# Eun0/XMC-GAN

Hardware: AMD Instinct MI355X
Metric: images/sec per G+D step (higher is better)
Workload: dtype bf16; 1 GPU; 256x256 COCO-shaped synthetic batch, 256 images per GPU, one full G+D iteration (D step + G step + Adam x2), df_gan_damsm_nomagp.yml; per_gpu_batch=256, global_batch=256, image_size=256, cfg=df_gan_damsm_nomagp.yml, parallelism=dp1, hipgraph=True, losses_finite=True, workload_name=headline

## Files before the change

### include/xmc_gan_hip.h

```cpp
#ifndef XMC_GAN_HIP_H
#define XMC_GAN_HIP_H

#include <stdint.h>

#ifdef __cplusplus
extern "C" {
#endif

#define XMC_ABI_VERSION 12

enum { XMC_BF16 = 0, XMC_F32 = 1 };
enum { XMC_HALF_IS_BF16 = 0, XMC_HALF_IS_F16 = 1 };
enum { XMC_ACT_NONE = 0, XMC_ACT_LRELU = 1, XMC_ACT_TANH = 2, XMC_ACT_RELU = 3 };
enum { XMC_EINVAL = -1, XMC_EALIGN = -2, XMC_ESHAPE = -3 };

#define XMC_MAX_TAPS 16
#define XMC_MAX_CLASSES 4

typedef struct XmcConvDesc {
    const void* src;
    const void* wpk;
    void* dst;
    const float* bias;
    const void* res;
// ... 38 lines not shown
const char* xmc_last_kernel(void);
int xmc_set_fixed_order(int on);
int xmc_set_prezeroed(int on);

int64_t xmc_conv_splitk_ws_bytes(const XmcConvDesc* d);

int xmc_conv_igemm(const XmcConvDesc* d, void* stream);

int xmc_conv_wgrad(const XmcConvDesc* d , float* dwp, void* stream);
#define XMC_BIAS_REPLICAS 16
int xmc_conv_wgrad_bias(const XmcConvDesc* d, float* dwp, float* dbias, void* stream);

int xmc_pack_weight(const float* w, void* wpk, int Co, int Ci, int KH, int KW, int rows_pad, int cols_pad,
                    int transpose , int dtype, const int32_t* row_perm , void* stream);
int xmc_pack_weight_grouped(const float* w, void* wpk, int Co, int Ci, int KH, int KW, int rows_pad, int cols_pad, int transpose,
                            int dtype, const int32_t* row_perm, int groups, void* stream);
int xmc_unpack_wgrad_grouped(const float* dwp, float* gw, int Co, int Ci, int KH, int KW, int rows_pad, int cols_pad,
                             const float* scale_dev, const int32_t* row_perm, int accumulate, int groups, void* stream);
#define XMC_PACK_MULTI_MAX 48
typedef struct XmcPackJob {
    const float* w;
    void* wpk;
    const int32_t* row_perm;
    int32_t Co, Ci, KHW, rows_pad, cols_pad, transpose, dtype, groups, upconv;
    int32_t lo;
} XmcPackJob;
int xmc_pack_weight_multi(const XmcPackJob* jobs , int njobs, void* stream);
int xmc_pack_weight_upconv(const float* w, void* wpk, int Co, int Ci, int rows_pad, int cols_pad, int transpose, int dtype,
                           void* stream);
int xmc_unpack_wgrad(const float* dwp, float* gw, int Co, int Ci, int KH, int KW, int rows_pad, int cols_pad,
                     const float* scale_dev, const int32_t* row_perm, int accumulate, void* stream);
int xmc_unpack_wgrad_bias(const float* dwp, float* gw, int Co, int Ci, int KH, int KW, int rows_pad, int cols_pad,
                          const float* scale_dev, const int32_t* row_perm, int accumulate,
                          const float* gb_replicas, float* gb, int CD, void* stream);
int xmc_unpack_wgrad_bias_dot(const float* dwp, float* gw, int Co, int Ci, int KH, int KW, int rows_pad, int cols_pad,
                              const float* scale_dev, const int32_t* row_perm, int accumulate,
                              const float* gb_replicas, float* gb, int CD, const float* bias_dot, float* dot, void* stream);

int xmc_nchw_to_nhwc8(const float* src , void* dst , int N, int C, int H, int W,
                      int dtype, void* stream);
int xmc_nhwc8_to_nchw(const void* src , float* dst , int N, int C, int H, int W,
                      int dtype, void* stream);

int xmc_lrelu(const void* x, void* y, int64_t n, float slope, int dtype, void* stream);
int xmc_lrelu_mask(const void* dy, const void* ref, void* dx, int64_t n, float slope, int dtype, void* stream);
int xmc_tanh(const void* x, void* y, int64_t n, int dtype, void* stream);
int xmc_signmask_apply(const void* dy, const void* bits, void* dx, int64_t n, float slope, int dtype, void* stream);
int xmc_conv_pw1x1_masked_src(const XmcConvDesc* d, const void* src_bits, void* src_masked, float slope, void* stream);
int xmc_conv_pw1x1_split(const XmcConvDesc* d, void* stream);
int xmc_conv_ptile_bits(const XmcConvDesc* d, void* stream);
int xmc_conv_ptile_scimg(const XmcConvDesc* d, void* stream);
int xmc_conv_wgrad_bits(const XmcConvDesc* d, float* dwp, void* stream);
int xmc_tanh_bwd(const void* dy, const void* y, void* dx, int64_t n, int dtype, void* stream);
int xmc_axpby(const void* a, const void* b, const float* alpha_dev, void* y, int64_t n, int dtype, void* stream);
int xmc_axpby_up(const void* a, const void* b, const float* alpha_dev, void* y, int N, int H, int W, int C, int dtype, void* stream);
int xmc_axpby_up_lrelu(const void* a, const void* b, const float* alpha_dev, void* y, int N, int H, int W, int C, int dtype, void* stream);
int xmc_scale(const void* x, const float* alpha_dev, void* y, int64_t n, int dtype, void* stream);
int xmc_dot(const void* a, const void* b, float* out, int64_t n, int dtype, void* stream);
enum { XMC_GP_BIAS = 1, XMC_GP_RELU = 2, XMC_GP_MASK = 4, XMC_GP_ATOMIC = 8 };
typedef struct XmcGemmProblem {
    const float* A;
    const float* B;
    const float* bias;
    const float* mask;
    float* C;
    float* rowsum;
    int32_t M, N, K;
    int32_t sa_i, sa_r, sb_j, sb_r;
    int32_t flags;
    int32_t tile0;
    int32_t reserved;
} XmcGemmProblem;
int xmc_gemm_group(const XmcGemmProblem* problems, int nproblems, void* stream);
int xmc_embedding_gather(const int64_t* ids, const float* table, float* out, int64_t n_tokens, int dim, int64_t vocab, void* stream);
int xmc_gru_bidir(const float* xproj, const float* w_hh, const float* b_hn, const int32_t* lens, float* words, float* sent, int B, int T,
                  int H, void* stream);
int xmc_lstm_bidir(const float* xproj, const float* w_hh, const int32_t* lens, float* words, float* sent, int B, int T, int H,
                   void* stream);
int xmc_spectral_sigma(const float* W, float* u, float* v, float* scratch, float* sig, float* w_eff, int R, int C, int training,
                       float eps, void* stream);
int xmc_spectral_bwd(const float* g, const float* W, const float* u, const float* v, const float* sig, float* dot, float* dW,
                     int R, int C, void* stream);
int xmc_scale_mask_dot(const void* dy, const void* ref, const float* alpha_dev, void* g, float* dot, int64_t n, int dtype, void* stream);
int xmc_axpby_bwd(const void* dy, const void* b, const float* alpha_dev, void* db, void* da, float* dot,
                  int N, int H, int W, int C, int up, const void* ymask , int dtype, void* stream);
int xmc_colsum(const void* x, float* out, int64_t rows, int C, int dtype, void* stream);
int xmc_avgpool2(const void* x, void* y, int N, int H, int W, int C, int dtype, void* stream);
int xmc_upsample2(const void* x, void* y, int N, int H, int W, int C, float scale, int dtype, void* stream);
int xmc_sumpool2(const void* x, void* y, int N, int H, int W, int C, float scale, int dtype, void* stream);
int xmc_global_avgpool(const void* x, void* y, int N, int HW, int C, int dtype, int out_dtype, void* stream);
int xmc_global_avgpool_bwd(const void* dy, void* dx, int N, int HW, int C, int dtype, int in_dtype, void* stream);

int xmc_affine2_lrelu_fwd(const void* x, const float* g0, const float* b0, const float* g1, const float* b1,
                          void* y, int N, int HW, int C, int dtype, void* stream);
int xmc_affine2_lrelu_bwd(const void* x, const void* dy, const float* g0, const float* b0, const float* g1,
                          const float* b1, void* dx, float* dg0, float* db0, float* dg1, float* db1,
                          int N, int HW, int C, int dtype, void* stream);

int xmc_affine2_act_fwd(const void* x, const float* g0, const float* b0, const float* g1, const float* b1,
                        void* y, int N, int HW, int C, float slope, int dtype, void* stream);
int xmc_affine2_act_bwd(const void* x, const void* dy, const float* g0, const float* b0, const float* g1,
                        const float* b1, void* dx, float* dg0, float* db0, float* dg1, float* db1,
                        int N, int HW, int C, float slope, int dtype, void* stream);
int xmc_affine2_act_bwd_acc(const void* x, const void* dy, const float* g0, const float* b0, const float* g1,
                            const float* b1, void* dx, float* dg0, float* db0, float* dg1, float* db1, const void* dx_in,
                            int N, int HW, int C, float slope, int dtype, void* stream);
// ... 131 lines not shown
```

### xmc-gan_amd/lib.py

```python
import ctypes as C
import os

HERE = os.path.dirname(os.path.abspath(__file__))
LIB_PATH = os.environ.get("XMC_LIB_PATH", os.path.join(HERE, "libxmc_gan_hip.so"))
LIB_PATH_F16 = os.environ.get("XMC_LIB_PATH_F16", os.path.join(HERE, "libxmc_gan_hip_f16.so"))
ABI_VERSION = 12

BF16, F32 = 0, 1
H16 = BF16
ACT_NONE, ACT_LRELU, ACT_TANH, ACT_RELU = 0, 1, 2, 3
MAX_TAPS, MAX_CLASSES = 16, 4

vp, i32, i64, f32 = C.c_void_p, C.c_int32, C.c_int64, C.c_float


class ConvDesc(C.Structure):
    _fields_ = [("src", vp), ("wpk", vp), ("dst", vp), ("bias", vp), ("res", vp), ("alpha_dev", vp),
                ("N", i32), ("SH", i32), ("SW", i32), ("CS", i32),
                ("DH", i32), ("DW", i32), ("CD", i32),
                ("MH", i32), ("MW", i32), ("SA", i32), ("DA", i32), ("src_shift", i32),
                ("ntaps", i32), ("nclass", i32), ("CDw", i32), ("act", i32), ("dtype", i32), ("out_dtype", i32),
                ("dh", (C.c_int8 * MAX_TAPS) * MAX_CLASSES), ("dw", (C.c_int8 * MAX_TAPS) * MAX_CLASSES),
                ("wi", (C.c_int8 * MAX_TAPS) * MAX_CLASSES),
                ("dph", C.c_int8 * MAX_CLASSES), ("dpw", C.c_int8 * MAX_CLASSES),
# ... 2 lines not shown
                ("splitk_ws", vp), ("splitk_ws_bytes", C.c_int64), ("wpk_lo", vp)]


GEMM_PROBLEM = [("A", "u8"), ("B", "u8"), ("bias", "u8"), ("mask", "u8"), ("C", "u8"), ("rowsum", "u8"),
                ("M", "i4"), ("N", "i4"), ("K", "i4"), ("sa_i", "i4"), ("sa_r", "i4"), ("sb_j", "i4"), ("sb_r", "i4"),
                ("flags", "i4"), ("tile0", "i4"), ("reserved", "i4")]
GP_BIAS, GP_RELU, GP_MASK, GP_ATOMIC = 1, 2, 4, 8


class PackJob(C.Structure):
    _fields_ = [("w", vp), ("wpk", vp), ("row_perm", vp), ("Co", i32), ("Ci", i32), ("KHW", i32), ("rows_pad", i32),
                ("cols_pad", i32), ("transpose", i32), ("dtype", i32), ("groups", i32), ("upconv", i32), ("lo", i32)]


class AdamEntry(C.Structure):
    _fields_ = [("param", vp), ("grad", vp), ("m", vp), ("v", vp), ("step", vp), ("n", i64)]


class EmaEntry(C.Structure):
    _fields_ = [("shadow", vp), ("param", vp), ("n", i64)]


_SIGS = {
    "xmc_abi_version": [],
    "xmc_half_format": [],
    "xmc_last_kernel": [],
    "xmc_set_fixed_order": [i32],
    "xmc_set_prezeroed": [i32],
    "xmc_conv_splitk_ws_bytes": [vp],
    "xmc_conv_igemm": [C.POINTER(ConvDesc), vp],
    "xmc_conv_wgrad": [C.POINTER(ConvDesc), vp, vp],
    "xmc_conv_wgrad_bias": [C.POINTER(ConvDesc), vp, vp, vp],
    "xmc_pack_weight": [vp, vp, i32, i32, i32, i32, i32, i32, i32, i32, vp, vp],
    "xmc_pack_weight_grouped": [vp, vp, i32, i32, i32, i32, i32, i32, i32, i32, vp, i32, vp],
    "xmc_pack_weight_upconv": [vp, vp, i32, i32, i32, i32, i32, i32, vp],
    "xmc_pack_weight_multi": [C.POINTER(PackJob), i32, vp],
    "xmc_axpby_up": [vp, vp, vp, vp, i32, i32, i32, i32, i32, vp],
    "xmc_unpack_wgrad": [vp, vp, i32, i32, i32, i32, i32, i32, vp, vp, i32, vp],
    "xmc_unpack_wgrad_grouped": [vp, vp, i32, i32, i32, i32, i32, i32, vp, vp, i32, i32, vp],
    "xmc_unpack_wgrad_bias": [vp, vp, i32, i32, i32, i32, i32, i32, vp, vp, i32, vp, vp, i32, vp],
    "xmc_unpack_wgrad_bias_dot": [vp, vp, i32, i32, i32, i32, i32, i32, vp, vp, i32, vp, vp, i32, vp, vp, vp],
    "xmc_nchw_to_nhwc8": [vp, vp, i32, i32, i32, i32, i32, vp],
    "xmc_nhwc8_to_nchw": [vp, vp, i32, i32, i32, i32, i32, vp],
    "xmc_lrelu": [vp, vp, i64, f32, i32, vp],
    "xmc_lrelu_mask": [vp, vp, vp, i64, f32, i32, vp],
    "xmc_tanh": [vp, vp, i64, i32, vp],
    "xmc_signmask_apply": [vp, vp, vp, i64, f32, i32, vp],
    "xmc_conv_pw1x1_masked_src": [C.POINTER(ConvDesc), vp, vp, f32, vp],
    "xmc_conv_pw1x1_split": [C.POINTER(ConvDesc), vp],
    "xmc_conv_ptile_bits": [C.POINTER(ConvDesc), vp],
    "xmc_conv_ptile_scimg": [C.POINTER(ConvDesc), vp],
    "xmc_conv_wgrad_bits": [C.POINTER(ConvDesc), vp, vp],
    "xmc_tanh_bwd": [vp, vp, vp, i64, i32, vp],
    "xmc_axpby": [vp, vp, vp, vp, i64, i32, vp],
    "xmc_scale_mask_dot": [vp, vp, vp, vp, vp, i64, i32, vp],
    "xmc_axpby_bwd": [vp, vp, vp, vp, vp, vp, i32, i32, i32, i32, i32, vp, i32, vp],
    "xmc_axpby_up_lrelu": [vp, vp, vp, vp, i32, i32, i32, i32, i32, vp],
    "xmc_scale": [vp, vp, vp, i64, i32, vp],
    "xmc_dot": [vp, vp, vp, i64, i32, vp],
    "xmc_gemm_group": [vp, i32, vp],
    "xmc_embedding_gather": [vp, vp, vp, i64, i32, i64, vp],
    "xmc_lstm_bidir": [vp, vp, vp, vp, vp, i32, i32, i32, vp],
    "xmc_gru_bidir": [vp, vp, vp, vp, vp, vp, i32, i32, i32, vp],
    "xmc_spectral_sigma": [vp, vp, vp, vp, vp, vp, i32, i32, i32, f32, vp],
    "xmc_spectral_bwd": [vp, vp, vp, vp, vp, vp, vp, i32, i32, vp],
    "xmc_colsum": [vp, vp, i64, i32, i32, vp],
    "xmc_avgpool2": [vp, vp, i32, i32, i32, i32, i32, vp],
    "xmc_upsample2": [vp, vp, i32, i32, i32, i32, f32, i32, vp],
    "xmc_sumpool2": [vp, vp, i32, i32, i32, i32, f32, i32, vp],
    "xmc_global_avgpool": [vp, vp, i32, i32, i32, i32, i32, vp],
    "xmc_global_avgpool_bwd": [vp, vp, i32, i32, i32, i32, i32, vp],
    "xmc_affine2_act_fwd": [vp, vp, vp, vp, vp, vp, i32, i32, i32, f32, i32, vp],
    "xmc_affine2_act_bwd": [vp, vp, vp, vp, vp, vp, vp, vp, vp, vp, vp, i32, i32, i32, f32, i32, vp],
    "xmc_affine2_act_bwd_acc": [vp, vp, vp, vp, vp, vp, vp, vp, vp, vp, vp, vp, i32, i32, i32, f32, i32, vp],
    "xmc_affine2_act_bwd_dot": [vp, vp, vp, vp, vp, vp, vp, vp, vp, vp, vp, vp, vp, vp, i32, i32, i32, f32, i32, vp],
    "xmc_affine2_act_bwd_dot_pool": [vp, vp, vp, vp, vp, vp, vp, vp, vp, vp, vp, vp, vp, vp, vp, i32, i32, i32, i32, f32, i32, vp],
    "xmc_affine2_lrelu_fwd": [vp, vp, vp, vp, vp, vp, i32, i32, i32, i32, vp],
    "xmc_affine2_lrelu_bwd": [vp, vp, vp, vp, vp, vp, vp, vp, vp, vp, vp, i32, i32, i32, i32, vp],
    "xmc_groupnorm_fwd": [vp, vp, vp, vp, vp, vp, i32, i32, i32, i32, f32, f32, i32, vp],
    "xmc_groupnorm_bwd": [vp, vp, vp, vp, vp, vp, vp, vp, vp, i32, i32, i32, i32, f32, i32, vp],
    "xmc_attn_pool_ws_floats": [i32, i32],
    "xmc_attn_pool_fwd": [vp, vp, vp, vp, vp, vp, i32, i32, i32, i32, i32, f32, i32, vp],
    "xmc_attn_pool_bwd": [vp, vp, vp, vp, vp, vp, vp, vp, vp, i32, i32, i32, i32, i32, f32, i32, vp],
    "xmc_attn_pool_bwd_acc": [vp, vp, vp, vp, vp, vp, vp, vp, vp, vp, i32, i32, i32, i32, i32, f32, i32, vp],
    "xmc_word_pool_fwd": [vp, vp, vp, vp, i32, i32, i32, i32, i32, i32, vp],
    "xmc_word_pool_bwd": [vp, vp, vp, vp, vp, vp, i32, i32, i32, i32, i32, i32, vp],
    "xmc_gvec_fwd": [vp, vp, vp, vp, vp, i32, i32, i32, i32, i32, vp],
    "xmc_gvec_bwd": [vp, vp, vp, vp, vp, vp, vp, vp, i32, i32, i32, i32, i32, vp],
    "xmc_reasoner_fwd": [vp, vp, vp, vp, vp, vp, i32, f32, f32, vp, vp, vp, i32, vp],
    "xmc_reasoner_bwd": [vp, vp, vp, vp, vp, vp, i32, vp, vp, vp, vp, vp, i32, vp],
    "xmc_word_ctx_fwd": [vp, vp, vp, vp, vp, i32, i32, vp],
    "xmc_word_ctx_bwd": [vp, vp, vp, vp, vp, vp, i32, i32, vp],
    "xmc_word_keys_fwd": [vp, vp, vp, f32, vp, vp, i32, i32, vp],
    "xmc_word_keys_bwd": [vp, vp, vp, vp, vp, vp, vp, vp, i32, i32, vp],
    "xmc_contrastive_ws_bytes": [i32, i32],
    "xmc_contrastive_fwd": [vp, vp, vp, vp, i32, i32, vp, vp, vp],
    "xmc_contrastive_bwd": [vp, vp, vp, vp, i32, i32, vp, vp, vp, vp, vp],
    "xmc_cosine_scores": [vp, vp, i32, i32, vp, vp, vp],
    "xmc_hinge_fwd": [vp, i32, f32, vp, i64, i32, vp],
    "xmc_hinge_bwd": [vp, i32, f32, vp, vp, i64, i32, vp],
    "xmc_cast": [vp, vp, i64, i32, i32, vp],
    "xmc_concept_query_fwd": [vp, vp, vp, vp, vp, vp, i32, i32, f32, vp],
    "xmc_concept_query_bwd": [vp, vp, vp, vp, vp, vp, vp, vp, vp, vp, i32, i32, f32, vp],
    "xmc_concept_query_fwd_multi": [vp, vp, vp, vp, i32, vp, vp, i32, i32, f32, vp],
    "xmc_concept_query_bwd_multi": [vp, vp, vp, i32, vp, vp, vp, vp, vp, vp, i32, i32, f32, vp],
    "xmc_concept_gquery_fwd": [vp, vp, vp, vp, vp, vp, i32, f32, vp],
# ... 83 lines not shown
```

### xmc-gan_amd/ops/_engine.py

```python
import ctypes as C
import weakref
import torch
from .. import lib as L
from .. import prof
from ._config import (
    _DEBUG_DISPATCH, _code, _nbytes, _need_cuda, _p, _st, _weights_epoch, bump_weights_epoch, chan_pad, pad_to)


class ConvGeom:

    __slots__ = ("cin", "cout", "k", "s", "p", "row_perm", "_perm_dev", "groups")

    def __init__(self, cin, cout, k=1, s=1, p=0, row_perm=None, groups=1):
        assert k * k <= L.MAX_TAPS and k % s == 0
        assert cin % groups == 0 and cout % groups == 0
        self.cin, self.cout, self.k, self.s, self.p = cin, cout, k, s, p
        self.groups = groups
        self.row_perm = row_perm
        self._perm_dev = None

    def out_hw(self, h, w):
        return (h + 2 * self.p - self.k) // self.s + 1, (w + 2 * self.p - self.k) // self.s + 1

    def perm_dev(self, device):
# ... 506 lines not shown

def _pool_key(t):
    return (t.data_ptr(), tuple(t.shape), t.dtype)


def _pooled_put(dx, dxp):
    _pooled_grads[_pool_key(dx)] = (dx, dx._version, dxp)


def _pooled_take(dz):
    ent = _pooled_grads.pop(_pool_key(dz), None)
    if ent is None:
        return None
    dx, ver, dxp = ent
    same = dx.untyped_storage().data_ptr() == dz.untyped_storage().data_ptr() and dx.stride() == dz.stride() and dx._version == ver
    return dxp if same else None


def _conv_wgrad_raw(x, dy, geom, scale=None, up=False, want_bias=False, bias_dot=None, dot=None):
    staged = dy if isinstance(dy, _StagedMask) else None
    if staged is not None:
        dy = staged.dy
    _need_cuda(x, dy)
    N, H, W, CS = x.shape
    _, OH, OW, CDy = dy.shape
    assert x.dtype == dy.dtype, (x.dtype, dy.dtype)
    rows = pad_to(CDy, 32)
    dwp = _arena.zeros((geom.k * geom.k, rows, CS), x.device)
    gb = _arena.zeros((16, CDy), x.device) if want_bias else None
    d = L.ConvDesc()
    d.src, d.dst = x.data_ptr(), dy.data_ptr()
    d.N, d.SH, d.SW, d.CS = N, H, W, CS
    d.DH, d.DW, d.CD = OH, OW, CDy
    d.MH, d.MW, d.SA, d.DA, d.src_shift = OH, OW, geom.s, 1, 1 if up else 0
    d.ntaps, d.nclass, d.CDw = geom.k * geom.k, 1, rows
    d.dtype, d.out_dtype = _code(x.dtype), L.F32
    d.groups = geom.groups
    _fill_taps(d, 0, [(kh - geom.p, kw - geom.p, kh * geom.k + kw) for kh in range(geom.k) for kw in range(geom.k)])
    rc = 1
    if staged is not None and not want_bias:
        d.mask_bits = staged.bits.data_ptr()
        with prof.launch("wgrad_kernel (conv weight gradient, MFMA + split-K atomics)", 2.0 * N * OH * OW * geom.cout * geom.cin * geom.k * geom.k,
                         f"wgrad+bits {x.dtype} N{N} {H}x{W} {geom.cin}->{geom.cout} k{geom.k}s{geom.s}", _nbytes(x, dy, dwp)):
            rc = L.load().xmc_conv_wgrad_bits(C.byref(d), _p(dwp), _st())
        if rc not in (0, 1):
            L.check(rc, "xmc_conv_wgrad_bits")
        d.mask_bits = None
    if rc == 1:
        if staged is not None:
            d.dst = staged.materialised().data_ptr()
        with prof.launch("wgrad_kernel (conv weight gradient, MFMA + split-K atomics)", 2.0 * N * OH * OW * geom.cout * geom.cin * geom.k * geom.k,
                         f"wgrad {x.dtype} N{N} {H}x{W} {geom.cin}->{geom.cout} k{geom.k}s{geom.s}", _nbytes(x, dy, dwp)):
            L.check(L.load().xmc_conv_wgrad_bias(C.byref(d), _p(dwp), _p(gb), _st()), "xmc_conv_wgrad")
    gw = torch.empty((geom.cout, geom.cin // geom.groups, geom.k, geom.k), dtype=torch.float32, device=x.device)
    if want_bias:
        assert geom.groups == 1
        gbs = torch.empty(CDy, dtype=torch.float32, device=x.device)
        assert (bias_dot is None) == (dot is None)
        L.call("xmc_unpack_wgrad_bias_dot", _p(dwp), _p(gw), geom.cout, geom.cin, geom.k, geom.k, rows, CS, _p(scale),
               _p(geom.perm_dev(x.device)), 0, _p(gb), _p(gbs), CDy, _p(bias_dot), _p(dot), _st())
        return gw, gbs
    assert bias_dot is None
    L.call("xmc_unpack_wgrad_grouped", _p(dwp), _p(gw), geom.cout, geom.cin, geom.k, geom.k, rows, CS, _p(scale),
           _p(geom.perm_dev(x.device)), 0, geom.groups, _st())
    return gw


def _axpby_bwd_fused(dy, b, alpha, up, ymask=None, want_db=True):
    dy = dy.contiguous()
    N, OH, OW, Cc = dy.shape
    H, W = (OH // 2, OW // 2) if up else (OH, OW)
    al = alpha.detach().reshape(-1).float()
    db = torch.empty_like(dy) if want_db else None
    da = torch.empty((N, H, W, Cc), dtype=dy.dtype, device=dy.device) if (up or ymask is not None) else None
    dot = _zeros_f32_out(1, dy.device)
    L.call("xmc_axpby_bwd", _p(dy), _p(b), _p(al), _p(db), _p(da), _p(dot), N, H, W, Cc, 1 if up else 0, _p(ymask), _code(dy.dtype), _st())
    return da, db, dot.reshape(alpha.shape).to(alpha.dtype)


def _affine_fwd_raw(x, ps, slope):
    N, H, W, Cc = x.shape
    for t in ps:
        assert t.shape == (N, Cc), (t.shape, (N, Cc))
    y = torch.empty_like(x)
    ptrs = [_p(t) for t in ps] + ([] if len(ps) == 4 else [None, None])
    L.call("xmc_affine2_act_fwd", _p(x), *ptrs, _p(y), N, H * W, Cc, float(slope), _code(x.dtype), _st())
    return y


def _affine_bwd_raw(x, dy, ps, slope, dx_acc=None, alpha=None, dot=None, want_sumpool=False):
    N, H, W, Cc = x.shape
    dx = torch.empty_like(x)
    if dx_acc is not None:
        dx_acc = dx_acc.contiguous()
        assert dx_acc.shape == x.shape and dx_acc.dtype == x.dtype
    nred = len(ps)
    red = _zeros_f32((nred, N, Cc), x.device)
    ptrs = [_p(t) for t in ps] + ([] if nred == 4 else [None, None])
    rptrs = [_p(red[i]) for i in range(nred)] + ([] if nred == 4 else [None, None])
    assert (alpha is None) == (dot is None)
    dxp = torch.empty((N, H // 2, W // 2, Cc), dtype=x.dtype, device=x.device) if want_sumpool else None
    L.call("xmc_affine2_act_bwd_dot_pool", _p(x), _p(dy), *ptrs, _p(dx), *rptrs, _p(dx_acc), _p(alpha), _p(dot), _p(dxp), N, H, W, Cc,
           float(slope), _code(x.dtype), _st())
    return (dx, red, dxp) if want_sumpool else (dx, red)


def compose_dstem(w_img, b_img, w0, ws, bs):
    F = torch.nn.functional
    co, mid = w0.shape[0], w0.shape[1]
    w0, b_img = w0.float(), b_img.float()
    wie = F.pad(w_img.float(), (0, 0, 0, 0, 0, 8 - w_img.shape[1]))
    wa = F.conv_transpose2d(w0, wie)
    box = torch.full((1, 1, 2, 2), 0.25, dtype=torch.float32, device=w_img.device)
    wp = F.conv_transpose2d(wie.reshape(mid * 8, 1, 3, 3), box).reshape(mid, 8, 4, 4)
    wb = torch.einsum("om,mcab->ocab", ws.float()[:, :, 0, 0], wp)
    w = torch.cat((wa, F.pad(wb, (1, 1, 1, 1)))).permute(0, 2, 3, 1).reshape(2 * co, 36, 8)
    ba = torch.einsum("omhw,m->o", w0, b_img)
    bb = ws.float()[:, :, 0, 0] @ b_img + (bs.float() if bs is not None else 0.0)
# ... 85 lines not shown
```

### xmc-gan_amd/ops/_nodes_conv.py

```python
import ctypes as C
import numpy as np
import torch
from .. import lib as L
from ._config import _code, _p, _skip_wgrad, _st, act_dtype, pad_to
from ._engine import (
    _affine_bwd_raw, _affine_fwd_raw, _axpby_bwd_fused, _conv1x1_pair_raw, _conv_dgrad_raw, _conv_fwd_raw, _conv_wgrad_raw,
    _pooled_take, _upconv_dgrad_raw, _upconv_fwd_raw, _zeros_f32, _zeros_f32_out)
from ._nodes_leaf import CastFn, ColSumFn, MaskFn, TanhBwdFn


def _bias_padded(b, geom, permute=False):
    if b is None:
        return None
    bp = b.detach().float()
    if permute and geom.row_perm is not None:
        bp = bp.index_select(0, geom.perm_dev(b.device).long())
    cd_p = pad_to(geom.cout, 8)
    if bp.numel() < cd_p:
        bp = torch.nn.functional.pad(bp, (0, cd_p - bp.numel()))
    return bp.contiguous()


def _act_bwd(dy, y, act, dtype):
    dy = dy.contiguous()
    if act in (L.ACT_LRELU, L.ACT_RELU):
        dy = MaskFn.apply(dy, y, 0.2 if act == L.ACT_LRELU else 0.0)
    elif act == L.ACT_TANH:
        dy = TanhBwdFn.apply(dy, y)
    return dy if dy.dtype == dtype else CastFn.apply(dy, dtype)


def _wgrad_bias_raw(ctx, x, dy, w, geom, scale=None, up=False):
    dw = db = None
    if not _skip_wgrad():
        want_b = ctx.has_b and ctx.needs_input_grad[2]
        if ctx.needs_input_grad[1]:
            r = _conv_wgrad_raw(x, dy, geom, scale=scale, up=up, want_bias=want_b)
            dw, db = r if want_b else (r, None)
            dw = dw.view(w.shape)
        elif want_b:
            db = ColSumFn.apply(dy)
            if scale is not None:
                db = db * scale
        if db is not None:
            db = db[: geom.cout]
    return dw, db


class ConvFn(torch.autograd.Function):

    @staticmethod
    def forward(ctx, x, w, b, geom, act, out_dtype, want_pool=False, out=None, pair=False):
        x = x.contiguous()
        assert out is None or out._version == 0, "ConvFn(out=): the destination must be a fresh tensor"
        bp = _bias_padded(b, geom, permute=True)
        if pair and x.dtype != torch.float32 and act == L.ACT_NONE and not want_pool and out is None:
            y = _conv1x1_pair_raw(x, w, bp, geom, out_dtype)
        else:
            y = _conv_fwd_raw(x, w, bp, geom, act, out_dtype, want_pool=want_pool, out=out)
        yp = None
# ... 147 lines not shown
        ctx.save_for_backward(h, w, res, gamma)
        return y

    @staticmethod
    @torch.autograd.function.once_differentiable
    def backward(ctx, dy):
        h, w, res, gamma = ctx.saved_tensors
        geom = ctx.geom
        dy = dy.contiguous()
        al = gamma.detach().reshape(-1).float()
        dsc, _, dgamma = _axpby_bwd_fused(dy, res, gamma, up=True, want_db=False)
        dh = _conv_dgrad_raw(dy, w, geom, (h.shape[1], h.shape[2]), h.dtype, alpha=al) if ctx.needs_input_grad[0] else None
        dw, db = _wgrad_bias_raw(ctx, h, dy, w, geom, scale=al)
        return dh, dw, db, None, (dsc if ctx.needs_input_grad[4] else None), (dgamma if ctx.needs_input_grad[5] else None)


def conv_axpby_up(h, w, b, geom, sc_lo, gamma):
    return ConvAxpbyUpFn.apply(h, w, b, geom, sc_lo, gamma)


class GBlockEndFn(torch.autograd.Function):

    @staticmethod
    def forward(ctx, h1, g0, b0, g1, b1, w2, b2, geom2, sc_lo, gamma, w_out=None, b_out=None, geom_out=None, nhwc_dst=None):
        h1, sc_lo = h1.contiguous(), sc_lo.contiguous()
        ps = [t.contiguous().float() for t in (g0, b0, g1, b1)]
        h2 = _affine_fwd_raw(h1, ps, 0.2)
        al = gamma.detach().reshape(-1).float()
        tail = w_out is not None
        y = _conv_fwd_raw(h2, w2, _bias_padded(b2, geom2), geom2, L.ACT_NONE, h2.dtype, res=sc_lo, alpha=al, res_mode=2,
                          round_act=True, post_act=L.ACT_LRELU if tail else L.ACT_NONE)
        img = None
        if tail:
            assert nhwc_dst is None or nhwc_dst._version == 0, "GBlockEndFn(nhwc_dst=): the destination must be a fresh tensor"
            img = _conv_fwd_raw(y, w_out, _bias_padded(b_out, geom_out), geom_out, L.ACT_TANH, y.dtype, out=nhwc_dst)
        ctx.geom2, ctx.geom_out, ctx.tail = geom2, geom_out, tail
        ctx.has_b2, ctx.has_bo = b2 is not None, b_out is not None
        ctx.save_for_backward(h1, *ps, h2, w2, b2, gamma, y if tail else None, w_out, img)
        return img if tail else y

    @staticmethod
    @torch.autograd.function.once_differentiable
    def backward(ctx, dy):
        h1, g0, b0, g1, b1, h2, w2, b2, gamma, y, w_out, img = ctx.saved_tensors
        geom2, geom_out = ctx.geom2, ctx.geom_out
        dt = h1.dtype
        N, H, W, _ = h2.shape
        dy = dy.contiguous()
        if dy.dtype != dt:
            dy = dy.to(dt)
        skip_w = _skip_wgrad()
        dw_out = db_out = None
        if ctx.tail:
            dpre = torch.empty_like(dy)
            L.call("xmc_tanh_bwd", _p(dy), _p(img), _p(dpre), dy.numel(), _code(dt), _st())
            if not skip_w:
                r = _conv_wgrad_raw(y, dpre, geom_out, want_bias=ctx.has_bo)
                dw_out, db_out = r if ctx.has_bo else (r, None)
                dw_out = dw_out.view(w_out.shape)
                if db_out is not None:
                    db_out = db_out[: geom_out.cout]
            dz, dsc = _conv_dgrad_raw(dpre, w_out, geom_out, (H, W), dt, mask=y, want_sumpool=True)
        else:
            dz = dy
            dsc = _pooled_take(dz)
            if dsc is None:
                dsc = torch.empty((N, H // 2, W // 2, dz.shape[3]), dtype=dt, device=dz.device)
                L.call("xmc_sumpool2", _p(dz), _p(dsc), N, H, W, dz.shape[3], 1.0, _code(dt), _st())
        al = gamma.detach().reshape(-1).float()
        dot = _zeros_f32_out(1, dz.device)
        dw2 = db2 = None
        if ctx.has_b2:
            bdot = _bias_padded(b2, geom2)
            dw2, db2 = _conv_wgrad_raw(h2, dz, geom2, scale=al, want_bias=True, bias_dot=bdot, dot=dot)
            dw2, db2 = dw2.view(w2.shape), db2[: geom2.cout]
        elif not skip_w:
            dw2 = _conv_wgrad_raw(h2, dz, geom2, scale=al).view(w2.shape)
        dh2u = _conv_dgrad_raw(dz, w2, geom2, (H, W), dt)
        dh1, red = _affine_bwd_raw(h1, dh2u, (g0, b0, g1, b1), 0.2, alpha=al, dot=dot)
        dgamma = dot.reshape(gamma.shape).to(gamma.dtype)
        if skip_w:
            dw2 = db2 = None
        return (dh1, red[0], red[1], red[2], red[3], dw2, db2, None, dsc, dgamma, dw_out, db_out, None, None)


def g_block_end(h1, mod4, c2w, c2b, geom2, sc_lo, gamma, tail=None, nhwc_dst=None):
    if tail is None:
        return GBlockEndFn.apply(h1, *mod4, c2w, c2b, geom2, sc_lo, gamma)
    return GBlockEndFn.apply(h1, *mod4, c2w, c2b, geom2, sc_lo, gamma, tail[0], tail[1], tail[2], nhwc_dst)


def conv2d(x, w, b, geom, act=L.ACT_NONE, out_dtype=None, want_pool=False, out=None, pair=False):
    return ConvFn.apply(x, w, b, geom, act, out_dtype or x.dtype, want_pool, out, pair)


def linear(x, w, b, geom, act=L.ACT_NONE, out_dtype=None):
    y = ConvFn.apply(x.contiguous().view(x.shape[0], 1, 1, x.shape[1]), w, b, geom, act, out_dtype or x.dtype)
    return y.view(x.shape[0], -1)


def _gemm_group(tab):
    L.call("xmc_gemm_group", C.c_void_p(tab.ctypes.data), len(tab), _st())


def _offsets(sizes):
    off = np.zeros(len(sizes) + 1, dtype=np.int64)
    np.cumsum(sizes, out=off[1:])
    return off


class CondMLPBankFn(torch.autograd.Function):

    @staticmethod
    def forward(ctx, c, *params):
        assert len(params) % 4 == 0 and c.dtype == torch.float32 and c.is_cuda
# ... 171 lines not shown
```

Measured before the change: 5980 images/s.

## Fuse generator tail backward: tanh-bwd, conv dgrad, mask, sumpool, wgrad in one kernel

Adds a single HIP kernel for the generator's output tail backward. In one tiled pass it applies the tanh backward, computes the 3x3 conv input gradient with MFMA, applies the lrelu mask, writes the sum-pooled shortcut gradient, and accumulates the weight and bias gradients. This replaces three separate launches and the round trip of the intermediate dpre tensor through memory. The old path remains as a fallback for unsupported shapes or dtypes, at the cost of a large specialized kernel that relies on atomics for the weight gradient.

```diff
diff --git a/include/xmc_gan_hip.h b/include/xmc_gan_hip.h
--- a/include/xmc_gan_hip.h
+++ b/include/xmc_gan_hip.h
@@ -114,6 +114,8 @@
 int xmc_conv_ptile_scimg(const XmcConvDesc* d, void* stream);
 int xmc_conv_wgrad_bits(const XmcConvDesc* d, float* dwp, void* stream);
 int xmc_tanh_bwd(const void* dy, const void* y, void* dx, int64_t n, int dtype, void* stream);
+int xmc_gtail_bwd(const void* dy, const void* img, const void* y, const void* wpk_t, void* dz, void* dsc, float* dwp, float* dbias,
+                  int N, int H, int W, int dtype, void* stream);
 int xmc_axpby(const void* a, const void* b, const float* alpha_dev, void* y, int64_t n, int dtype, void* stream);
 int xmc_axpby_up(const void* a, const void* b, const float* alpha_dev, void* y, int N, int H, int W, int C, int dtype, void* stream);
 int xmc_axpby_up_lrelu(const void* a, const void* b, const float* alpha_dev, void* y, int N, int H, int W, int C, int dtype, void* stream);
diff --git a/xmc-gan_amd/csrc/gtail.hip b/xmc-gan_amd/csrc/gtail.hip
--- /dev/null
+++ b/xmc-gan_amd/csrc/gtail.hip
@@ -0,0 +1,233 @@
+#include "common.h"
+
+namespace {
+
+constexpr int GT_TH = 8, GT_TW = 32, GT_PH = GT_TH + 2, GT_PW = GT_TW + 2, GT_NPIX = GT_PH * GT_PW;
+constexpr int GT_XS = 96;
+constexpr int GT_YIT = (GT_NPIX * 4 + 255) / 256;
+
+template <bool WG>
+__global__ __launch_bounds__(256, 3) void gtail_bwd_kernel(const u32x4* __restrict__ dy16, const u32x4* __restrict__ img16,
+                                                          const u32x4* __restrict__ y16, const u32x4* __restrict__ w16,
+                                                          bf16x8* __restrict__ dz8, bf16x8* __restrict__ dsc8, float* __restrict__ dwp,
+                                                          float* __restrict__ dbias, int H, int W, int tiles_y, int tiles_x, int ntiles) {
+    constexpr int TH = GT_TH, TW = GT_TW, PW = GT_PW, XS = GT_XS, KS = 3, NS = 4, MAXI = 5, NITEMS = 18;
+    __shared__ __attribute__((aligned(16))) unsigned char dp[GT_NPIX * 16];
+    __shared__ __attribute__((aligned(16))) unsigned char yp[GT_NPIX * XS];
+    const int tid = threadIdx.x, lane = tid & 63, wm = tid >> 6;
+    const int fr = lane & 15, fc = lane >> 4;
+
+    u32x4 wf[KS][2];
+    int toff[KS];
+#pragma unroll
+    for (int ks = 0; ks < KS; ++ks) {
+        const int tap = ks * 4 + fc;
+        const bool live = tap < 9;
+        const int tt = live ? tap : 0;
+        toff[ks] = ((2 - tt / 3) * PW + (2 - tt % 3)) * 16;
+#pragma unroll
+        for (int j = 0; j < 2; ++j) {
+            const int lrow = (fr >> 2) * 8 + j * 4 + (fr & 3);
+            wf[ks][j] = live ? w16[tt * 32 + lrow] : u32x4{0, 0, 0, 0};
+        }
+    }
+    int psrc[2];
+    unsigned halo = 0;
+    const bool pin1 = tid + 256 < GT_NPIX;
+#pragma unroll
+    for (int it = 0; it < 2; ++it) {
+        const int pp = tid + it * 256;
+        const int py = pp / PW, px = pp - py * PW;
+        const bool in = pp < GT_NPIX;
+        psrc[it] = in ? (py - 1) * W + (px - 1) : 0;
+        halo |= (!in ? 0u : ((py < 1 ? 1u : 0u) | (py > TH ? 2u : 0u) | (px < 1 ? 4u : 0u) | (px > TW ? 8u : 0u))) << (4 * it);
+    }
+    const int ych = tid & 3;
+    int yoff[GT_YIT];
+    unsigned yhalo = 0, yin = 0;
+#pragma unroll
+    for (int it = 0; it < GT_YIT; ++it) {
+        const int pp = (tid + it * 256) >> 2;
+        const int py = pp / PW, px = pp - py * PW;
+        const bool in = pp < GT_NPIX;
+        yin |= in ? (1u << it) : 0u;
+        yoff[it] = in ? ((py - 1) * W + (px - 1)) * 4 + ych : 0;
+        yhalo |= (!in ? 0u : ((py < 1 ? 1u : 0u) | (py > TH ? 2u : 0u) | (px < 1 ? 4u : 0u) | (px > TW ? 8u : 0u))) << (4 * it);
+    }
+    const int pbase0 = (wm * 2 * PW + fr) * 16, eoff0 = (wm * 2 * W + fr) * 4 + fc, moff0 = ((wm * 2 + 1) * PW + fr + 1) * XS + fc * 16;
+    const int q4 = fr >> 2, pp4 = fr & 3;
+    int itoff[MAXI];
+#pragma unroll
+    for (int j = 0; j < MAXI; ++j) {
+        const int item = wm + j * NS;
+        const int ib = item < NITEMS ? item / 9 : 0, tap = item < NITEMS ? item % 9 : 0;
+        itoff[j] = ((tap / 3) * PW + tap % 3) * XS + ib * 32;
+    }
+    const int nv = __builtin_amdgcn_readfirstlane(wm < NITEMS - 4 * NS ? MAXI : MAXI - 1);
+    const unsigned char* const afrag = dp + (PW + 1 + 4 * fc + q4) * 16 + pp4 * 8;
+    const unsigned char* const bfrag = yp + (4 * fc + q4) * XS + pp4 * 8;
+    f32x4 acc[WG ? MAXI : 1];
+#pragma unroll
+    for (int j = 0; j < (WG ? MAXI : 1); ++j) acc[j] = f32x4{0.f, 0.f, 0.f, 0.f};
+    const bool bias_wave = __builtin_amdgcn_readfirstlane(WG && dbias != nullptr && wm == 2);
+
+    const int tpi = tiles_y * tiles_x;
+    u32x4 pdy[2], pim[2], pyv[GT_YIT];
+    unsigned okbits = 0;
+    auto issue = [&](int tile) {
+        const int n = __builtin_amdgcn_readfirstlane(tile / tpi), trem = tile - n * tpi;
+        const int ty = __builtin_amdgcn_readfirstlane(trem / tiles_x), tx = trem - ty * tiles_x;
+        const int base = (n * H + ty * TH) * W + tx * TW;
+        const unsigned border = (ty == 0 ? 1u : 0u) | (ty == tiles_y - 1 ? 2u : 0u) | (tx == 0 ? 4u : 0u) | (tx == tiles_x - 1 ? 8u : 0u);
+        okbits = 0;
+#pragma unroll
+        for (int it = 0; it < 2; ++it) {
+            const bool ok = (((halo >> (4 * it)) & 15u) & border) == 0;
+            const size_t idx = (size_t)(base + (ok ? psrc[it] : 0));
+            pdy[it] = dy16[idx];
+            pim[it] = img16[idx];
+            okbits |= ok ? (1u << it) : 0u;
+        }
+        const u32x4* __restrict__ yb = y16 + (size_t)base * 4;
+#pragma unroll
+        for (int it = 0; it < GT_YIT; ++it) {
+            const bool ok = (((yhalo >> (4 * it)) & 15u) & border) == 0;
+            pyv[it] = yb[ok ? yoff[it] : 0];
+            okbits |= ok ? (4u << it) : 0u;
+        }
+    };
+    const XcdWalk xw = xmc_xcd_walk(ntiles);
+    int tile = xw.first;
+    if (tile < xw.end) issue(tile);
+    for (; tile < xw.end; tile += xw.step) {
+        const int n = tile / tpi, trem = tile - n * tpi;
+        const int ty = trem / tiles_x, tx = trem - ty * tiles_x;
+        __syncthreads();
+#pragma unroll
+        for (int it = 0; it < 2; ++it) {
+            const bf16x8 a = __builtin_bit_cast(bf16x8, pdy[it]), b = __builtin_bit_cast(bf16x8, pim[it]);
+            bf16x8 o;
+#pragma unroll
+            for (int k = 0; k < 8; ++k) {
+                const float g = (float)a[k], t = (float)b[k];
+                o[k] = (xmc_h16)(g * (1.f - t * t));
+            }
+            u32x4 v = __builtin_bit_cast(u32x4, o);
+            if (!((okbits >> it) & 1)) v = u32x4{0, 0, 0, 0};
+            if (it == 0 || pin1) *reinterpret_cast<u32x4*>(dp + (tid + it * 256) * 16) = v;
+        }
+#pragma unroll
+        for (int it = 0; it < GT_YIT; ++it) {
+            u32x4 v = pyv[it];
+            if (!((okbits >> (2 + it)) & 1)) v = u32x4{0, 0, 0, 0};
+            if ((yin >> it) & 1) *reinterpret_cast<u32x4*>(yp + ((tid + it * 256) >> 2) * XS + ych * 16) = v;
+        }
+        __syncthreads();
+        if (tile + xw.step < xw.end) issue(tile + xw.step);
+
+        const int dbase = ((n * H + ty * TH) * W + tx * TW) * 4;
+#pragma unroll
+        for (int ip = 0; ip < 2; ++ip) {
+            float fin[2][8];
+#pragma unroll
+            for (int h = 0; h < 2; ++h) {
+                const int i = ip + 2 * h;
+                f32x4 dacc[2] = {f32x4{0.f, 0.f, 0.f, 0.f}, f32x4{0.f, 0.f, 0.f, 0.f}};
+#pragma unroll
+                for (int ks = 0; ks < KS; ++ks) {
+                    const u32x4 pf = *reinterpret_cast<const u32x4*>(dp + pbase0 + ((i >> 1) * PW + (i & 1) * 16) * 16 + toff[ks]);
+#pragma unroll
+                    for (int j = 0; j < 2; ++j)
+                        dacc[j] = XMC_MFMA_16x16x32(__builtin_bit_cast(bf16x8, wf[ks][j]), __builtin_bit_cast(bf16x8, pf), dacc[j], 0, 0, 0);
+                }
+                const bf16x8 mk = *reinterpret_cast<const bf16x8*>(yp + moff0 + ((i >> 1) * PW + (i & 1) * 16) * XS);
+                bf16x8 o;
+#pragma unroll
+                for (int q = 0; q < 4; ++q) {
+                    const float x0 = dacc[0][q] + 0.f, x1 = dacc[1][q] + 0.f;
+                    o[q] = (xmc_h16)(x0 * lrelu_slope((float)mk[q]));
+                    o[4 + q] = (xmc_h16)(x1 * lrelu_slope((float)mk[4 + q]));
+                }
+                dz8[dbase + eoff0 + ((i >> 1) * W + (i & 1) * 16) * 4] = o;
+#pragma unroll
+                for (int q = 0; q < 8; ++q) fin[h][q] = (float)o[q];
+            }
+            const int prow = ty * (TH / 2) + wm, pcol = tx * (TW / 2) + ((ip * 16 + fr) >> 1);
+            bf16x8 o;
+#pragma unroll
+            for (int q = 0; q < 8; ++q) {
+                float sm = fin[0][q] + fin[1][q];
+                sm += xmc_xor1(sm);
+                o[q] = (xmc_h16)(1.f * sm);
+            }
+            if ((fr & 1) == 0) dsc8[((n * (H >> 1) + prow) * (W >> 1) + pcol) * 4 + fc] = o;
+        }
+
+        if constexpr (WG) {
+            int zq = 0;
+            asm volatile("" : "+v"(zq));
+            const unsigned char* const afr = afrag + zq;
+            const unsigned char* const bfr = bfrag + zq;
+            const xmc_h16 one = (xmc_h16)1.f;
+            const bf16x8 ones = bf16x8{one, one, one, one, one, one, one, one};
+#pragma unroll 2
+            for (int r = 0; r < TH; ++r) {
+                const unsigned char* const ab = afr + r * PW * 16;
+                const bf16x4 alo = xmc_ds_read_tr16(ab), ahi = xmc_ds_read_tr16(ab + 16 * 16);
+                const bf16x8 af = bf16x8{alo[0], alo[1], alo[2], alo[3], ahi[0], ahi[1], ahi[2], ahi[3]};
+#pragma unroll
+                for (int j = 0; j < MAXI; ++j) {
+                    if (j < nv) {
+                        const unsigned char* const bb = bfr + r * PW * XS + itoff[j];
+                        const bf16x4 blo = xmc_ds_read_tr16(bb), bhi = xmc_ds_read_tr16(bb + 16 * XS);
+                        const bf16x8 bf = bf16x8{blo[0], blo[1], blo[2], blo[3], bhi[0], bhi[1], bhi[2], bhi[3]};
+                        acc[j] = XMC_MFMA_16x16x32(af, bf, acc[j], 0, 0, 0);
+                    } else if (bias_wave) {
+                        acc[j] = XMC_MFMA_16x16x32(af, ones, acc[j], 0, 0, 0);
+                    }
+                }
+            }
+        }
+    }
+
+    if constexpr (WG) {
+        if (bias_wave && fr == 0 && fc < 2) {
+#pragma unroll
+            for (int rr = 0; rr < 4; ++rr) atomicAdd(&dbias[(blockIdx.x & (XMC_BIAS_REPLICAS - 1)) * 8 + fc * 4 + rr], acc[MAXI - 1][rr]);
+        }
+#pragma unroll
+        for (int j = 0; j < MAXI; ++j) {
+            const int item = wm + j * NS;
+            if (item < NITEMS && fc < 2) {
+                const int ib = item / 9, tap = item - ib * 9;
+#pragma unroll
+                for (int rr = 0; rr < 4; ++rr) atomicAdd(&dwp[(tap * 32 + fc * 4 + rr) * 32 + ib * 16 + fr], acc[j][rr]);
+            }
+        }
+    }
+}
+
+}
+
+extern "C" int xmc_gtail_bwd(const void* dy, const void* img, const void* y, const void* wpk_t, void* dz, void* dsc, float* dwp,
+                             float* dbias, int N, int H, int W, int dtype, void* stream) {
+    if (!dy || !img || !y || !wpk_t || !dz || !dsc || (dbias && !dwp)) return XMC_EINVAL;
+    if (N < 1 || H < 1 || W < 1) return XMC_ESHAPE;
+    static const bool off = xmc_debug_off("no_gtail_fused");
+    if (off || dtype != XMC_BF16 || H % GT_TH != 0 || W % GT_TW != 0) return 1;
+    if ((int64_t)N * H * W * 32 >= (1ll << 31)) return 1;
+    const int tiles_y = H / GT_TH, tiles_x = W / GT_TW, ntiles = N * tiles_y * tiles_x;
+    int gx = 256 * 3;
+    if (gx > ntiles) gx = ntiles;
+    hipStream_t st = reinterpret_cast<hipStream_t>(stream);
+    const dim3 grid(xmc_ab_grid(gx)), block(256);
+    if (dwp)
+        hipLaunchKernelGGL((gtail_bwd_kernel<true>), grid, block, 0, st, (const u32x4*)dy, (const u32x4*)img, (const u32x4*)y, (const u32x4*)wpk_t,
+                           (bf16x8*)dz, (bf16x8*)dsc, dwp, dbias, H, W, tiles_y, tiles_x, ntiles);
+    else
+        hipLaunchKernelGGL((gtail_bwd_kernel<false>), grid, block, 0, st, (const u32x4*)dy, (const u32x4*)img, (const u32x4*)y, (const u32x4*)wpk_t,
+                           (bf16x8*)dz, (bf16x8*)dsc, nullptr, nullptr, H, W, tiles_y, tiles_x, ntiles);
+    xmc_note_kernel(dwp ? "gtail_bwd_kernel<true>" : "gtail_bwd_kernel<false>");
+    XMC_LAUNCH_CHECK();
+    return 0;
+}
diff --git a/xmc-gan_amd/lib.py b/xmc-gan_amd/lib.py
--- a/xmc-gan_amd/lib.py
+++ b/xmc-gan_amd/lib.py
@@ -78,6 +78,7 @@
     "xmc_conv_ptile_scimg": [C.POINTER(ConvDesc), vp],
     "xmc_conv_wgrad_bits": [C.POINTER(ConvDesc), vp, vp],
     "xmc_tanh_bwd": [vp, vp, vp, i64, i32, vp],
+    "xmc_gtail_bwd": [vp, vp, vp, vp, vp, vp, vp, vp, i32, i32, i32, i32, vp],
     "xmc_axpby": [vp, vp, vp, vp, i64, i32, vp],
     "xmc_scale_mask_dot": [vp, vp, vp, vp, vp, i64, i32, vp],
     "xmc_axpby_bwd": [vp, vp, vp, vp, vp, vp, i32, i32, i32, i32, i32, vp, i32, vp],
diff --git a/xmc-gan_amd/ops/_engine.py b/xmc-gan_amd/ops/_engine.py
--- a/xmc-gan_amd/ops/_engine.py
+++ b/xmc-gan_amd/ops/_engine.py
@@ -582,18 +582,47 @@
         with prof.launch("wgrad_kernel (conv weight gradient, MFMA + split-K atomics)", 2.0 * N * OH * OW * geom.cout * geom.cin * geom.k * geom.k,
                          f"wgrad {x.dtype} N{N} {H}x{W} {geom.cin}->{geom.cout} k{geom.k}s{geom.s}", _nbytes(x, dy, dwp)):
             L.check(L.load().xmc_conv_wgrad_bias(C.byref(d), _p(dwp), _p(gb), _st()), "xmc_conv_wgrad")
-    gw = torch.empty((geom.cout, geom.cin // geom.groups, geom.k, geom.k), dtype=torch.float32, device=x.device)
-    if want_bias:
+    return _unpack_wgrad(dwp, gb, geom, rows, CS, CDy, scale, bias_dot, dot)
+
+
+def _unpack_wgrad(dwp, gb, geom, rows, CS, CDy, scale=None, bias_dot=None, dot=None):
+    gw = torch.empty((geom.cout, geom.cin // geom.groups, geom.k, geom.k), dtype=torch.float32, device=dwp.device)
+    if gb is not None:
         assert geom.groups == 1
-        gbs = torch.empty(CDy, dtype=torch.float32, device=x.device)
+        gbs = torch.empty(CDy, dtype=torch.float32, device=dwp.device)
         assert (bias_dot is None) == (dot is None)
         L.call("xmc_unpack_wgrad_bias_dot", _p(dwp), _p(gw), geom.cout, geom.cin, geom.k, geom.k, rows, CS, _p(scale),
-               _p(geom.perm_dev(x.device)), 0, _p(gb), _p(gbs), CDy, _p(bias_dot), _p(dot), _st())
+               _p(geom.perm_dev(dwp.device)), 0, _p(gb), _p(gbs), CDy, _p(bias_dot), _p(dot), _st())
         return gw, gbs
     assert bias_dot is None
     L.call("xmc_unpack_wgrad_grouped", _p(dwp), _p(gw), geom.cout, geom.cin, geom.k, geom.k, rows, CS, _p(scale),
-           _p(geom.perm_dev(x.device)), 0, geom.groups, _st())
+           _p(geom.perm_dev(dwp.device)), 0, geom.groups, _st())
     return gw
+
+
+def _gtail_bwd_raw(dy, img, y, w_out, geom, want_w, want_bias):
+    N, H, W, CS = y.shape
+    if (dy.dtype == torch.float32 or CS != 32 or dy.shape[3] != 8 or (geom.k, geom.s, geom.p, geom.groups) != (3, 1, 1, 1) or
+            geom.row_perm is not None or H % 8 or W % 32):
+        return None
+    _need_cuda(dy, img, y, w_out)
+    assert dy.shape == img.shape == (N, H, W, 8) and dy.dtype == img.dtype == y.dtype and geom.cin == 32
+    wpk = _packed_cached(w_out, geom, 1, dy.dtype)
+    dz = torch.empty_like(y)
+    dsc = torch.empty((N, H // 2, W // 2, CS), dtype=y.dtype, device=y.device)
+    dwp = _arena.zeros((9, 32, CS), y.device) if want_w else None
+    gb = _arena.zeros((16, 8), y.device) if want_w and want_bias else None
+    with prof.launch("gtail_bwd_kernel (generator tail backward, one pass)", 2.0 * N * H * W * geom.cout * geom.cin * 9 * (2 if want_w else 1),
+                     f"gtail bwd {dy.dtype} N{N} {H}x{W}", _nbytes(dy, img, y, dz, dsc)):
+        rc = L.load().xmc_gtail_bwd(_p(dy), _p(img), _p(y), _p(wpk), _p(dz), _p(dsc), _p(dwp), _p(gb), N, H, W, _code(dy.dtype), _st())
+    if rc == 1:
+        return None
+    L.check(rc, "xmc_gtail_bwd")
+    dw = db = None
+    if want_w:
+        r = _unpack_wgrad(dwp, gb, geom, 32, CS, 8)
+        dw, db = r if want_bias else (r, None)
+    return dz, dsc, dw, db
 
 
 def _axpby_bwd_fused(dy, b, alpha, up, ymask=None, want_db=True):
diff --git a/xmc-gan_amd/ops/_nodes_conv.py b/xmc-gan_amd/ops/_nodes_conv.py
--- a/xmc-gan_amd/ops/_nodes_conv.py
+++ b/xmc-gan_amd/ops/_nodes_conv.py
@@ -5,7 +5,7 @@
 from ._config import _code, _p, _skip_wgrad, _st, act_dtype, pad_to
 from ._engine import (
     _affine_bwd_raw, _affine_fwd_raw, _axpby_bwd_fused, _conv1x1_pair_raw, _conv_dgrad_raw, _conv_fwd_raw, _conv_wgrad_raw,
-    _pooled_take, _upconv_dgrad_raw, _upconv_fwd_raw, _zeros_f32, _zeros_f32_out)
+    _gtail_bwd_raw, _pooled_take, _upconv_dgrad_raw, _upconv_fwd_raw, _zeros_f32, _zeros_f32_out)
 from ._nodes_leaf import CastFn, ColSumFn, MaskFn, TanhBwdFn
 
 
@@ -259,15 +259,20 @@
         skip_w = _skip_wgrad()
         dw_out = db_out = None
         if ctx.tail:
-            dpre = torch.empty_like(dy)
-            L.call("xmc_tanh_bwd", _p(dy), _p(img), _p(dpre), dy.numel(), _code(dt), _st())
-            if not skip_w:
-                r = _conv_wgrad_raw(y, dpre, geom_out, want_bias=ctx.has_bo)
-                dw_out, db_out = r if ctx.has_bo else (r, None)
+            r = _gtail_bwd_raw(dy, img, y, w_out, geom_out, not skip_w, ctx.has_bo)
+            if r is not None:
+                dz, dsc, dw_out, db_out = r
+            else:
+                dpre = torch.empty_like(dy)
+                L.call("xmc_tanh_bwd", _p(dy), _p(img), _p(dpre), dy.numel(), _code(dt), _st())
+                if not skip_w:
+                    r = _conv_wgrad_raw(y, dpre, geom_out, want_bias=ctx.has_bo)
+                    dw_out, db_out = r if ctx.has_bo else (r, None)
+                dz, dsc = _conv_dgrad_raw(dpre, w_out, geom_out, (H, W), dt, mask=y, want_sumpool=True)
+            if dw_out is not None:
                 dw_out = dw_out.view(w_out.shape)
-                if db_out is not None:
-                    db_out = db_out[: geom_out.cout]
-            dz, dsc = _conv_dgrad_raw(dpre, w_out, geom_out, (H, W), dt, mask=y, want_sumpool=True)
+            if db_out is not None:
+                db_out = db_out[: geom_out.cout]
         else:
             dz = dy
             dsc = _pooled_take(dz)
```

Measured after the change: 6035 images/s, median of 6. About the same (+0.9%).
